# EsauPR/3d-pose-baseline

Measured on NVIDIA B200. Metric: poses/sec (fused MLP inference, bf16), higher is better.
Workload: dtype bf16

## Files before the change

3d-pose-baseline_b200/csrc/mlp_tc.cu:

```cuda
#include <cstdlib>

#include "common.cuh"
#include "ptx.cuh"

namespace p3d {

static std::atomic<unsigned long long> g_l2_set_aside[64];
int l2persist_acquire(int dev, size_t bytes) {
  if (dev < 0 || dev >= 64) return P3D_OK;
  if (g_l2_set_aside[dev].load(std::memory_order_acquire) >= bytes) return P3D_OK;
  P3D_CUDA(cudaDeviceSetLimit(cudaLimitPersistingL2CacheSize, bytes));
  g_l2_set_aside[dev].store(bytes, std::memory_order_release);
  return P3D_OK;
}
int l2persist_release(int dev) {
  if (dev < 0 || dev >= 64 || g_l2_set_aside[dev].load(std::memory_order_acquire) == 0) return P3D_OK;
  cudaCtxResetPersistingL2Cache();
  P3D_CUDA(cudaDeviceSetLimit(cudaLimitPersistingL2CacheSize, 0));
  g_l2_set_aside[dev].store(0, std::memory_order_release);
  return P3D_OK;
}

namespace tc {

using namespace ptx;

constexpr int BM = 128;
constexpr int BN = 256;
constexpr int BK = 64;
constexpr int A_BYTES = BM * BK * 2;
constexpr int OUT_BYTES = BM * 64 * 2;
constexpr int NTHREADS = 256;
constexpr int TMEM_COLS = 512;
constexpr int MAX_SLABS = 64;

template <int CG> struct Tile {
  static constexpr int STAGES = CG == 1 ? 4 : 6;
  static constexpr int BAR_BYTES = 1024;
  static constexpr int B_ROWS = BN / CG;
  static constexpr int B_BYTES = B_ROWS * BK * 2;
  static constexpr int SMEM_BYTES = 1024  + STAGES * (A_BYTES + B_BYTES) + OUT_BYTES + 2 * BN * 4 + BAR_BYTES;
  static_assert(SMEM_BYTES <= 232448, "exceeds the 227 KB of shared memory per CTA");
};

struct Params {
  int L;
  int nlayers;
  int out_n;
  int out_valid;
  int residual;
  int ntiles;
  long long B;
  long long act_half_rows;
  const float* bias;
  float* y;
};

__device__ __forceinline__ uint32_t pack_bf16x2(float a, float b) {
  __nv_bfloat162 v = __floats2bfloat162_rn(a, b);
  return *reinterpret_cast<uint32_t*>(&v);
}

__device__ __forceinline__ uint64_t desc_at(uint32_t smem_addr) {
  constexpr uint32_t hi = (1024u >> 4) | (1u << 14) | (2u << 29);
  const uint32_t lo = ((smem_addr >> 4) & 0x3FFFu) | (1u << 16);
  return (static_cast<uint64_t>(hi) << 32) | lo;
}

template <int CG>
__global__ void __launch_bounds__(NTHREADS, 1)
mlp_forward_tc_kernel(const __grid_constant__ CUtensorMap tm_x, const __grid_constant__ CUtensorMap tm_act,
                      const __grid_constant__ CUtensorMap tm_w, const __grid_constant__ CUtensorMap tm_wout,
                      const Params p) {
  using T = Tile<CG>;
  constexpr int STAGES = T::STAGES;
  constexpr int B_BYTES = T::B_BYTES;
  extern __shared__ uint8_t smem_raw[];
  uint8_t* smem = reinterpret_cast<uint8_t*>((reinterpret_cast<uintptr_t>(smem_raw) + 1023) & ~uintptr_t(1023));
  uint8_t* sA = smem;
  uint8_t* sB = smem + STAGES * A_BYTES;
  uint8_t* sOut = sB + STAGES * B_BYTES;
  float* sBiasAll = reinterpret_cast<float*>(sOut + OUT_BYTES);
  uint64_t* bars = reinterpret_cast<uint64_t*>(sBiasAll + 2 * BN);
  uint64_t* full = bars;
  uint64_t* empty = bars + STAGES;
  uint64_t* tfull = bars + 2 * STAGES;
  uint64_t* tempty = tfull + 2;
  uint64_t* stg_full = tempty + 2;
  uint64_t* stg_free = stg_full + 1;
  uint64_t* slab_done = stg_free + 1;
  uint32_t* tmem_slot = reinterpret_cast<uint32_t*>(slab_done + MAX_SLABS);

  const int warp = threadIdx.x >> 5;
  const int lane = threadIdx.x & 31;
  const uint32_t rank = (CG == 2) ? cluster_ctarank() : 0u;
  const bool leader = (rank == 0);
  const int group_id = blockIdx.x / CG, ngroups = gridDim.x / CG;
  const int ngtiles = (p.ntiles + CG - 1) / CG;

  if (threadIdx.x == 0) {
    tma_prefetch_desc(&tm_x); tma_prefetch_desc(&tm_act); tma_prefetch_desc(&tm_w); tma_prefetch_desc(&tm_wout);
    for (int s = 0; s < STAGES; ++s) { mbar_init(&full[s], 2); mbar_init(&empty[s], 1); }
    for (int a = 0; a < 2; ++a) { mbar_init(&tfull[a], 1); mbar_init(&tempty[a], 4 * CG); }
    mbar_init(stg_full, 4); mbar_init(stg_free, 1);
    for (int c = 0; c < MAX_SLABS; ++c) mbar_init(&slab_done[c], 1);
    fence_barrier_init();
  }
  if (warp == 2) {
    if (CG == 2) { tmem_alloc_2sm(tmem_slot, TMEM_COLS); tmem_relinquish_2sm(); }
    else { tmem_alloc(tmem_slot, TMEM_COLS); tmem_relinquish(); }
  }
  tc_fence_before();
  if (CG == 2) cluster_sync(); else __syncthreads();
  tc_fence_after();
  const uint32_t tmem_base = *tmem_slot;

  const int L = p.L;
  const int nlayers = p.nlayers;
  const int nk_hidden = L / BK;
  const int nchunks_hidden = L / BN;

  if (warp == 0 || warp == 2) {
    const bool prodA = (warp == 0);
    int stage = 0; uint32_t phase = 0; uint32_t dep_layers = 0;
    for (int gt = group_id; gt < ngtiles; gt += ngroups) {
      const int tile = gt * CG + static_cast<int>(rank);
      for (int l = 0; l < nlayers; ++l) {
        const bool first = (l == 0), last = (l == nlayers - 1);
        const int nk = first ? 1 : nk_hidden;
        const int nchunks = last ? 1 : nchunks_hidden;
        const CUtensorMap* tmA = first ? &tm_x : &tm_act;
        const int a_row = first ? tile * BM
                                : static_cast<int>(((l & 1) ? 0 : p.act_half_rows) + static_cast<long long>(blockIdx.x) * BM);
        const int b_rows = last ? p.out_n / CG : T::B_ROWS;
        const uint32_t bytes = prodA ? A_BYTES : b_rows * BK * 2;
        for (int c = 0; c < nchunks; ++c) {
          const int b_row = (last ? 0 : l * L + c * BN) + static_cast<int>(rank) * b_rows;
          for (int ks = 0; ks < nk; ++ks) {
            if (prodA && !first && c == 0) mbar_wait(&slab_done[ks], dep_layers & 1, 100 + l);
            mbar_wait(&empty[stage], phase ^ 1, 1);
            if (elect_one()) {
              if (CG == 1) {
                mbar_arrive_expect_tx(&full[stage], bytes);
                if (prodA) tma_load_2d_hint(sA + stage * A_BYTES, tmA, &full[stage], ks * BK, a_row, first ? kEvictFirst : kEvictLast);
                else       tma_load_2d_hint(sB + stage * B_BYTES, last ? &tm_wout : &tm_w, &full[stage], ks * BK, b_row, kEvictLast);
              } else {
                if (leader) mbar_arrive_expect_tx(&full[stage], 2 * bytes);
                if (prodA) tma_load_2d_2sm_hint(sA + stage * A_BYTES, tmA, &full[stage], ks * BK, a_row, first ? kEvictFirst : kEvictLast);
                else       tma_load_2d_2sm_hint(sB + stage * B_BYTES, last ? &tm_wout : &tm_w, &full[stage], ks * BK, b_row, kEvictLast);
              }
            }
            __syncwarp();
            if (++stage == STAGES) { stage = 0; phase ^= 1; }
          }
        }
        if (!first) ++dep_layers;
      }
    }
  } else if (warp == 1 && leader) {
    int stage = 0; uint32_t phase = 0; uint32_t q = 0;
    const uint32_t idesc_hidden = umma_idesc_bf16_f32(BM * CG, BN);
    const uint32_t idesc_out = umma_idesc_bf16_f32(BM * CG, p.out_n);
    const uint32_t a_base = smem_u32(sA), b_base = smem_u32(sB);
    for (int gt = group_id; gt < ngtiles; gt += ngroups) {
      for (int l = 0; l < nlayers; ++l) {
        const bool first = (l == 0), last = (l == nlayers - 1);
        const int nk = first ? 1 : nk_hidden;
        const int nchunks = last ? 1 : nchunks_hidden;
        const uint32_t idesc = last ? idesc_out : idesc_hidden;
        for (int c = 0; c < nchunks; ++c, ++q) {
          const uint32_t acc = q & 1, aphase = (q >> 1) & 1;
          mbar_wait(&tempty[acc], aphase ^ 1, 2);
          tc_fence_after();
          const uint32_t d_tmem = tmem_base + acc * BN;
          for (int ks = 0; ks < nk; ++ks) {
            mbar_wait(&full[stage], phase, 3);
            tc_fence_after();
            if (elect_one()) {
              const uint64_t ad = desc_at(a_base + stage * A_BYTES);
              const uint64_t bd = desc_at(b_base + stage * B_BYTES);
#pragma unroll
              for (int k = 0; k < BK / 16; ++k) {
                if (CG == 1) umma_bf16_ss(d_tmem, ad + 2 * k, bd + 2 * k, idesc, (ks | k) != 0 ? 1u : 0u);
                else         umma_bf16_ss_2sm(d_tmem, ad + 2 * k, bd + 2 * k, idesc, (ks | k) != 0 ? 1u : 0u);
              }
              if (CG == 1) {
                umma_commit(&empty[stage]);
                if (ks == nk - 1) umma_commit(&tfull[acc]);
              } else {
                umma_commit_2sm(&empty[stage], 0x3);
                if (ks == nk - 1) umma_commit_2sm(&tfull[acc], 0x3);
              }
            }
            __syncwarp();
            if (++stage == STAGES) { stage = 0; phase ^= 1; }
          }
        }
      }
    }
  } else if (warp == 3) {
    if (lane == 0) {
      uint32_t n = 0;
      for (int gt = group_id; gt < ngtiles; gt += ngroups) {
        for (int l = 0; l < nlayers - 1; ++l) {
          const bool to_p = (l == 0) || ((l & 1) == 0);
          const bool add_res = p.residual && l >= 2 && ((l & 1) == 0);
          const int drow = static_cast<int>((to_p ? 0 : p.act_half_rows) + static_cast<long long>(blockIdx.x) * BM);
          const int nsl = L / 64;
          for (int sl = 0; sl < nsl; ++sl, ++n) {
            mbar_wait(stg_full, n & 1, 6);
            if (add_res) tma_reduce_add_2d_hint(&tm_act, sOut, sl * 64, drow, kEvictLast);
            else         tma_store_2d_hint(&tm_act, sOut, sl * 64, drow, kEvictLast);
            tma_store_commit();
            tma_store_wait_read<0>();
            mbar_arrive(stg_free);
            if (sl > 0) { tma_store_wait<1>(); mbar_arrive(&slab_done[sl - 1]); }
          }
          tma_store_wait<0>();
          mbar_arrive(&slab_done[nsl - 1]);
        }
      }
    }
  } else if (warp >= 4) {
    const int ew = warp - 4;
    const int row = ew * 32 + lane;
    uint8_t* my_out = sOut + row * 128;
    uint32_t q = 0, nslab = 0;
    for (int gt = group_id; gt < ngtiles; gt += ngroups) {
      const int tile = gt * CG + static_cast<int>(rank);
      for (int l = 0; l < nlayers; ++l) {
        const bool last = (l == nlayers - 1);
        const int nchunks = last ? 1 : nchunks_hidden;
        for (int c = 0; c < nchunks; ++c, ++q) {
          const uint32_t acc = q & 1, aphase = (q >> 1) & 1;
          const int wrow0 = last ? (nlayers - 1) * L : l * L + c * BN;
          float* sBias = sBiasAll + (q & 1) * BN;
          sBias[row] = __ldg(p.bias + wrow0 + row);
          if (!last) sBias[row + 128] = __ldg(p.bias + wrow0 + row + 128);
          named_bar_sync(1, 128);
          mbar_wait(&tfull[acc], aphase, 4);
          tc_fence_after();
          const uint32_t taddr = tmem_base + (static_cast<uint32_t>(ew * 32) << 16) + acc * BN;
          if (!last) {
#pragma unroll 1
            for (int s = 0; s < BN / 64; ++s) {
              uint32_t v0[32], v1[32];
              tmem_ld_32x32b_x32(taddr + s * 64, v0);
              tmem_ld_32x32b_x32(taddr + s * 64 + 32, v1);
              tmem_ld_wait();
              if (s == BN / 64 - 1) {
                tc_fence_before();
                __syncwarp();
                if (lane == 0) { if (CG == 1) mbar_arrive(&tempty[acc]); else mbar_arrive_cluster(&tempty[acc], 0); }
              }
              uint32_t o[32];
              const float* bs = sBias + s * 64;
#pragma unroll
              for (int j = 0; j < 16; ++j) {
                o[j] = pack_bf16x2(fmaxf(__uint_as_float(v0[2 * j]) + bs[2 * j], 0.f),
                                   fmaxf(__uint_as_float(v0[2 * j + 1]) + bs[2 * j + 1], 0.f));
                o[16 + j] = pack_bf16x2(fmaxf(__uint_as_float(v1[2 * j]) + bs[32 + 2 * j], 0.f),
                                        fmaxf(__uint_as_float(v1[2 * j + 1]) + bs[32 + 2 * j + 1], 0.f));
              }
              mbar_wait(stg_free, (nslab & 1) ^ 1, 5);
#pragma unroll
              for (int j = 0; j < 8; ++j)
                *reinterpret_cast<uint4*>(my_out + ((j ^ (row & 7)) << 4)) = make_uint4(o[4 * j], o[4 * j + 1], o[4 * j + 2], o[4 * j + 3]);
              fence_proxy_async_smem();
              __syncwarp();
              if (lane == 0) mbar_arrive(stg_full);
              ++nslab;
            }
          } else {
            const long long grow = static_cast<long long>(tile) * BM + row;
            for (int g = 0; g < p.out_n / 16; ++g) {
              uint32_t v[16];
              tmem_ld_32x32b_x16(taddr + g * 16, v);
              tmem_ld_wait();
              if (grow < p.B) {
                float* yp = p.y + grow * p.out_valid + g * 16;
#pragma unroll
                for (int j = 0; j < 16; j += 2) {
                  const int col = g * 16 + j;
                  if (col + 1 < p.out_valid) {
                    float2 o2 = make_float2(__uint_as_float(v[j]) + sBias[col], __uint_as_float(v[j + 1]) + sBias[col + 1]);
                    __stcs(reinterpret_cast<float2*>(yp + j), o2);
                  } else if (col < p.out_valid) {
                    __stcs(yp + j, __uint_as_float(v[j]) + sBias[col]);
                  }
                }
              }
            }
            tc_fence_before();
            __syncwarp();
            if (lane == 0) { if (CG == 1) mbar_arrive(&tempty[acc]); else mbar_arrive_cluster(&tempty[acc], 0); }
          }
        }
      }
    }
  }

  tc_fence_before();
  if (CG == 2) cluster_sync(); else __syncthreads();
  if (warp == 2) {
    tc_fence_after();
    if (CG == 2) tmem_dealloc_2sm(tmem_base, TMEM_COLS); else tmem_dealloc(tmem_base, TMEM_COLS);
  }
}

constexpr int B_BYTES = BN * BK * 2;
__global__ void __launch_bounds__(128, 1)
umma_gemm_debug_kernel(const __grid_constant__ CUtensorMap tm_a, const __grid_constant__ CUtensorMap tm_w,
                       float* C, int N, int K) {
  extern __shared__ uint8_t smem_raw[];
  uint8_t* smem = reinterpret_cast<uint8_t*>((reinterpret_cast<uintptr_t>(smem_raw) + 1023) & ~uintptr_t(1023));
  uint8_t* sA = smem;
  uint8_t* sB = smem + A_BYTES;
  uint64_t* bar_full = reinterpret_cast<uint64_t*>(sB + B_BYTES);
  uint64_t* bar_mma = bar_full + 1;
  uint32_t* tmem_slot = reinterpret_cast<uint32_t*>(bar_mma + 1);
  const int warp = threadIdx.x >> 5, lane = threadIdx.x & 31;
  if (threadIdx.x == 0) { mbar_init(bar_full, 1); mbar_init(bar_mma, 1); fence_barrier_init(); }
  if (warp == 0) { tmem_alloc(tmem_slot, 256); tmem_relinquish(); }
  tc_fence_before(); __syncthreads(); tc_fence_after();
  const uint32_t tmem_base = *tmem_slot;
  if (threadIdx.x == 0) {
    const uint32_t idesc = umma_idesc_bf16_f32(128, N);
    for (int ks = 0; ks < K / BK; ++ks) {
      mbar_arrive_expect_tx(bar_full, A_BYTES + N * BK * 2);
      tma_load_2d(sA, &tm_a, bar_full, ks * BK, 0);
      tma_load_2d(sB, &tm_w, bar_full, ks * BK, 0);
      mbar_wait(bar_full, ks & 1, 10);
      tc_fence_after();
      for (int k = 0; k < BK / 16; ++k)
        umma_bf16_ss(tmem_base, umma_desc_k_sw128(smem_u32(sA) + k * 32), umma_desc_k_sw128(smem_u32(sB) + k * 32),
                     idesc, (ks | k) != 0 ? 1u : 0u);
      umma_commit(bar_mma);
      mbar_wait(bar_mma, ks & 1, 11);
    }
  }
  tc_fence_before(); __syncthreads(); tc_fence_after();
  const int row = warp * 32 + lane;
  for (int g = 0; g < N / 16; ++g) {
    uint32_t v[16];
    tmem_ld_32x32b_x16(tmem_base + (static_cast<uint32_t>(warp * 32) << 16) + g * 16, v);
    tmem_ld_wait();
    for (int j = 0; j < 16; ++j) C[row * N + g * 16 + j] = __uint_as_float(v[j]);
  }
  tc_fence_before(); __syncthreads();
  if (warp == 0) { tc_fence_after(); tmem_dealloc(tmem_base, 256); }
}

typedef CUresult (*EncodeTiledFn)(CUtensorMap*, CUtensorMapDataType, cuuint32_t, void*, const cuuint64_t*,
                                  const cuuint64_t*, const cuuint32_t*, const cuuint32_t*, CUtensorMapInterleave,
                                  CUtensorMapSwizzle, CUtensorMapL2promotion, CUtensorMapFloatOOBfill);

static EncodeTiledFn get_encode_fn() {
  static EncodeTiledFn fn = nullptr;
  if (!fn) {
    void* ptr = nullptr;
    cudaDriverEntryPointQueryResult qres;
    if (cudaGetDriverEntryPoint("cuTensorMapEncodeTiled", &ptr, cudaEnableDefault, &qres) != cudaSuccess ||
        qres != cudaDriverEntryPointSuccess)
      return nullptr;
    fn = reinterpret_cast<EncodeTiledFn>(ptr);
  }
  return fn;
}

static int make_tmap(CUtensorMap* out, const void* base, uint64_t rows, uint64_t cols, uint64_t pitch_elems,
                     uint32_t box_rows) {
  EncodeTiledFn fn = get_encode_fn();
  if (!fn) { set_error("cuTensorMapEncodeTiled entry point not available"); return P3D_ERR_CUDA; }
  cuuint64_t gdim[2] = {cols, rows};
  cuuint64_t gstride[1] = {pitch_elems * 2};
  cuuint32_t box[2] = {static_cast<cuuint32_t>(BK), box_rows};
  cuuint32_t estr[2] = {1, 1};
  CUresult r = fn(out, CU_TENSOR_MAP_DATA_TYPE_BFLOAT16, 2, const_cast<void*>(base), gdim, gstride, box, estr,
                  CU_TENSOR_MAP_INTERLEAVE_NONE, CU_TENSOR_MAP_SWIZZLE_128B, CU_TENSOR_MAP_L2_PROMOTION_L2_256B,
                  CU_TENSOR_MAP_FLOAT_OOB_FILL_NONE);
  if (r != CUDA_SUCCESS) { set_error("cuTensorMapEncodeTiled failed with CUresult %d", (int)r); return P3D_ERR_CUDA; }
  return P3D_OK;
}

template <int CG>
static int launch_forward(p3d_model* m, const __nv_bfloat16* xb, float* y, int64_t B, cudaStream_t st) {
  using T = Tile<CG>;
  const int L = m->L;
  const int ntiles = static_cast<int>((B + BM - 1) / BM);
  const int ngtiles = (ntiles + CG - 1) / CG;
  const int max_groups = m->num_sms / CG;
  const int grid = CG * (ngtiles < max_groups ? ngtiles : max_groups);
  const int nlayers = static_cast<int>(m->layers.size());
  const int out_n = (m->out_size + 15) / 16 * 16;
  CUtensorMap tm_x, tm_act, tm_w, tm_wout;
  P3D_TRY(make_tmap(&tm_x, xb, static_cast<uint64_t>(B), 64, 64, BM));
  P3D_TRY(make_tmap(&tm_act, m->act_scratch, 2ull * grid * BM, L, L, BM));
  P3D_TRY(make_tmap(&tm_w, m->wt_bf16, static_cast<uint64_t>(nlayers - 1) * L, m->kpad, m->kpad, T::B_ROWS));
  P3D_TRY(make_tmap(&tm_wout, m->wt_bf16 + static_cast<size_t>(nlayers - 1) * L * m->kpad, out_n, m->kpad, m->kpad, out_n / CG));
  Params p;
  p.L = L; p.nlayers = nlayers; p.out_n = out_n; p.out_valid = m->out_size; p.residual = m->cfg.residual;
  p.ntiles = ntiles; p.B = B; p.act_half_rows = static_cast<long long>(grid) * BM;
  p.bias = m->bias_fold; p.y = y;
  static PerDeviceOnce attr_set;
  if (attr_set.needed()) {
    P3D_CUDA(cudaFuncSetAttribute(mlp_forward_tc_kernel<CG>, cudaFuncAttributeMaxDynamicSharedMemorySize, T::SMEM_BYTES));
    attr_set.mark();
  }
  cudaLaunchConfig_t cfg{};
  cfg.gridDim = dim3(grid); cfg.blockDim = dim3(NTHREADS); cfg.dynamicSmemBytes = T::SMEM_BYTES; cfg.stream = st;
  cudaLaunchAttribute attr[2];
  attr[0].id = cudaLaunchAttributeClusterDimension;
  attr[0].val.clusterDim.x = CG; attr[0].val.clusterDim.y = 1; attr[0].val.clusterDim.z = 1;
  cfg.attrs = attr; cfg.numAttrs = 1;
  static const bool l2_persist = [] { const char* e = getenv("P3D_L2_PERSIST"); return !(e && e[0] == '0'); }();
  if (l2_persist) {
    int dev = 0, max_persist = 0, max_window = 0;
    P3D_CUDA(cudaGetDevice(&dev));
    P3D_CUDA(cudaDeviceGetAttribute(&max_persist, cudaDevAttrMaxPersistingL2CacheSize, dev));
    P3D_CUDA(cudaDeviceGetAttribute(&max_window, cudaDevAttrMaxAccessPolicyWindowSize, dev));
    const size_t scratch = sizeof(__nv_bfloat16) * 2ull * grid * BM * L;
    if (scratch <= static_cast<size_t>(max_persist) && scratch <= static_cast<size_t>(max_window)) {
      P3D_TRY(l2persist_acquire(dev, scratch));
      attr[1].id = cudaLaunchAttributeAccessPolicyWindow;
      attr[1].val.accessPolicyWindow.base_ptr = m->act_scratch;
      attr[1].val.accessPolicyWindow.num_bytes = scratch;
      attr[1].val.accessPolicyWindow.hitRatio = 1.0f;
      attr[1].val.accessPolicyWindow.hitProp = cudaAccessPropertyPersisting;
      attr[1].val.accessPolicyWindow.missProp = cudaAccessPropertyNormal;
      cfg.numAttrs = 2;
    }
  }
  cudaEvent_t e0 = nullptr, e1 = nullptr;
  if (prof::enabled()) prof::begin(st, &e0, &e1);
  P3D_CUDA(cudaLaunchKernelEx(&cfg, mlp_forward_tc_kernel<CG>, tm_x, tm_act, tm_w, tm_wout, p));
  P3D_LAUNCH_CHECK();
  if (e0) prof::end(st, e0, e1);
  return P3D_OK;
}

int forward_bf16(p3d_model* m, const __nv_bfloat16* xb, float* y, int64_t B, cudaStream_t st) {
  const int L = m->L;
  P3D_REQUIRE(L % BN == 0 && L / 64 <= MAX_SLABS, "bf16 tensor-core path needs linear_size %% 256 == 0 and <= 4096 (got %d)", L);
  if (m->act_grid < m->num_sms) {
    if (m->act_scratch) cudaFree(m->act_scratch);
    P3D_CUDA(cudaMalloc(&m->act_scratch, sizeof(__nv_bfloat16) * 2ull * m->num_sms * BM * L));
    m->act_grid = m->num_sms;
  }
  static int cg = -1;
  if (cg < 0) {
    const char* e = getenv("P3D_TC_CG");
    cg = (e && e[0] == '1') ? 1 : 2;
  }
  return cg == 1 ? launch_forward<1>(m, xb, y, B, st) : launch_forward<2>(m, xb, y, B, st);
}

int debug_umma_gemm(const void* A, const void* W, float* C, int N, int K, cudaStream_t st) {
  P3D_REQUIRE(N % 16 == 0 && N >= 16 && N <= 256 && K % 64 == 0 && K >= 64, "debug gemm: bad N=%d K=%d", N, K);
  CUtensorMap tm_a, tm_w;
  P3D_TRY(make_tmap(&tm_a, A, 128, K, K, 128));
  P3D_TRY(make_tmap(&tm_w, W, N, K, K, N));
  const int smem = 1024 + A_BYTES + B_BYTES + 64;
  P3D_CUDA(cudaFuncSetAttribute(umma_gemm_debug_kernel, cudaFuncAttributeMaxDynamicSharedMemorySize, smem));
  umma_gemm_debug_kernel<<<1, 128, smem, st>>>(tm_a, tm_w, C, N, K);
  P3D_LAUNCH_CHECK();
  return P3D_OK;
}

}
}
```

Before: 153.3 million.

## Widen epilogue to eight warps issuing their own TMA stores, drop store warp

Removes the dedicated TMA-store warp and the single shared output staging buffer. Eight epilogue warps now each own a small staging buffer and issue their own stores or reduce-adds per 32-row quarter, using a new 32-row tensor map. Each pair of warps splits the TMEM column slabs and software-pipelines the TMEM loads against the bias/ReLU/pack work. The goal is to take the store serialization and the stg_full/stg_free handshake off the critical path between layers. In exchange, pipeline stages drop by one to free shared memory, the thread count grows to 384, and optional clock64 stamp instrumentation is added behind an environment variable.

```diff
diff --git a/3d-pose-baseline_b200/csrc/mlp_tc.cu b/3d-pose-baseline_b200/csrc/mlp_tc.cu
--- a/3d-pose-baseline_b200/csrc/mlp_tc.cu
+++ b/3d-pose-baseline_b200/csrc/mlp_tc.cu
@@ -29,17 +29,20 @@
 constexpr int BN = 256;
 constexpr int BK = 64;
 constexpr int A_BYTES = BM * BK * 2;
-constexpr int OUT_BYTES = BM * 64 * 2;
-constexpr int NTHREADS = 256;
+constexpr int EPI_ROWS = 32;
+constexpr int STG_BYTES = EPI_ROWS * 64 * 2;
+constexpr int EPI_WARPS = 8;
+constexpr int NTHREADS = (4 + EPI_WARPS) * 32;
 constexpr int TMEM_COLS = 512;
 constexpr int MAX_SLABS = 64;
 
 template <int CG> struct Tile {
-  static constexpr int STAGES = CG == 1 ? 4 : 6;
+  static constexpr int STAGES = CG == 1 ? 3 : 5;
   static constexpr int BAR_BYTES = 1024;
   static constexpr int B_ROWS = BN / CG;
   static constexpr int B_BYTES = B_ROWS * BK * 2;
-  static constexpr int SMEM_BYTES = 1024  + STAGES * (A_BYTES + B_BYTES) + OUT_BYTES + 2 * BN * 4 + BAR_BYTES;
+  static constexpr int SMEM_BYTES = 1024  + STAGES * (A_BYTES + B_BYTES) + EPI_WARPS * STG_BYTES +
+                                    2 * BN * 4 + BAR_BYTES;
   static_assert(SMEM_BYTES <= 232448, "exceeds the 227 KB of shared memory per CTA");
 };
 
@@ -54,7 +57,19 @@
   long long act_half_rows;
   const float* bias;
   float* y;
+  unsigned long long* stamps;
 };
+
+constexpr int STAMP_SLOTS = 64;
+constexpr int STAMP_SPAN = 0;
+constexpr int STAMP_TILES = 1;
+constexpr int STAMP_EPI_STG = 2;
+constexpr int STAMP_EPI_TFULL = 3;
+constexpr int STAMP_MAX_LAYERS = 16;
+constexpr int STAMP_TEMPTY = 16;
+constexpr int STAMP_FULL = 32;
+constexpr int STAMP_SLAB = 48;
+__device__ __forceinline__ int stamp_layer(int l) { return l < STAMP_MAX_LAYERS ? l : STAMP_MAX_LAYERS - 1; }
 
 __device__ __forceinline__ uint32_t pack_bf16x2(float a, float b) {
   __nv_bfloat162 v = __floats2bfloat162_rn(a, b);
@@ -67,11 +82,11 @@
   return (static_cast<uint64_t>(hi) << 32) | lo;
 }
 
-template <int CG>
+template <int CG, bool STAMPS>
 __global__ void __launch_bounds__(NTHREADS, 1)
 mlp_forward_tc_kernel(const __grid_constant__ CUtensorMap tm_x, const __grid_constant__ CUtensorMap tm_act,
-                      const __grid_constant__ CUtensorMap tm_w, const __grid_constant__ CUtensorMap tm_wout,
-                      const Params p) {
+                      const __grid_constant__ CUtensorMap tm_act_st, const __grid_constant__ CUtensorMap tm_w,
+                      const __grid_constant__ CUtensorMap tm_wout, const Params p) {
   using T = Tile<CG>;
   constexpr int STAGES = T::STAGES;
   constexpr int B_BYTES = T::B_BYTES;
@@ -79,16 +94,14 @@
   uint8_t* smem = reinterpret_cast<uint8_t*>((reinterpret_cast<uintptr_t>(smem_raw) + 1023) & ~uintptr_t(1023));
   uint8_t* sA = smem;
   uint8_t* sB = smem + STAGES * A_BYTES;
-  uint8_t* sOut = sB + STAGES * B_BYTES;
-  float* sBiasAll = reinterpret_cast<float*>(sOut + OUT_BYTES);
+  uint8_t* sStg = sB + STAGES * B_BYTES;
+  float* sBiasAll = reinterpret_cast<float*>(sStg + EPI_WARPS * STG_BYTES);
   uint64_t* bars = reinterpret_cast<uint64_t*>(sBiasAll + 2 * BN);
   uint64_t* full = bars;
   uint64_t* empty = bars + STAGES;
   uint64_t* tfull = bars + 2 * STAGES;
   uint64_t* tempty = tfull + 2;
-  uint64_t* stg_full = tempty + 2;
-  uint64_t* stg_free = stg_full + 1;
-  uint64_t* slab_done = stg_free + 1;
+  uint64_t* slab_done = tempty + 2;
   uint32_t* tmem_slot = reinterpret_cast<uint32_t*>(slab_done + MAX_SLABS);
 
   const int warp = threadIdx.x >> 5;
@@ -97,13 +110,16 @@
   const bool leader = (rank == 0);
   const int group_id = blockIdx.x / CG, ngroups = gridDim.x / CG;
   const int ngtiles = (p.ntiles + CG - 1) / CG;
+  unsigned long long* stamps = STAMPS ? p.stamps + static_cast<size_t>(blockIdx.x) * STAMP_SLOTS : nullptr;
+  long long t_entry = 0;
+  if constexpr (STAMPS) t_entry = clock64();
 
   if (threadIdx.x == 0) {
-    tma_prefetch_desc(&tm_x); tma_prefetch_desc(&tm_act); tma_prefetch_desc(&tm_w); tma_prefetch_desc(&tm_wout);
+    tma_prefetch_desc(&tm_x); tma_prefetch_desc(&tm_act); tma_prefetch_desc(&tm_act_st);
+    tma_prefetch_desc(&tm_w); tma_prefetch_desc(&tm_wout);
     for (int s = 0; s < STAGES; ++s) { mbar_init(&full[s], 2); mbar_init(&empty[s], 1); }
-    for (int a = 0; a < 2; ++a) { mbar_init(&tfull[a], 1); mbar_init(&tempty[a], 4 * CG); }
-    mbar_init(stg_full, 4); mbar_init(stg_free, 1);
-    for (int c = 0; c < MAX_SLABS; ++c) mbar_init(&slab_done[c], 1);
+    for (int a = 0; a < 2; ++a) { mbar_init(&tfull[a], 1); mbar_init(&tempty[a], EPI_WARPS * CG); }
+    for (int c = 0; c < MAX_SLABS; ++c) mbar_init(&slab_done[c], 4);
     fence_barrier_init();
   }
   if (warp == 2) {
@@ -129,6 +145,7 @@
         const bool first = (l == 0), last = (l == nlayers - 1);
         const int nk = first ? 1 : nk_hidden;
         const int nchunks = last ? 1 : nchunks_hidden;
+        long long w_slab = 0;
         const CUtensorMap* tmA = first ? &tm_x : &tm_act;
         const int a_row = first ? tile * BM
                                 : static_cast<int>(((l & 1) ? 0 : p.act_half_rows) + static_cast<long long>(blockIdx.x) * BM);
@@ -137,7 +154,12 @@
         for (int c = 0; c < nchunks; ++c) {
           const int b_row = (last ? 0 : l * L + c * BN) + static_cast<int>(rank) * b_rows;
           for (int ks = 0; ks < nk; ++ks) {
-            if (prodA && !first && c == 0) mbar_wait(&slab_done[ks], dep_layers & 1, 100 + l);
+            if (prodA && !first && c == 0) {
+              long long t0 = 0;
+              if constexpr (STAMPS) t0 = clock64();
+              mbar_wait(&slab_done[ks], dep_layers & 1, 100 + l);
+              if constexpr (STAMPS) w_slab += clock64() - t0;
+            }
             mbar_wait(&empty[stage], phase ^ 1, 1);
             if (elect_one()) {
               if (CG == 1) {
@@ -155,6 +177,7 @@
           }
         }
         if (!first) ++dep_layers;
+        if constexpr (STAMPS) if (prodA && lane == 0 && w_slab) atomicAdd(stamps + STAMP_SLAB + stamp_layer(l), static_cast<unsigned long long>(w_slab));
       }
     }
   } else if (warp == 1 && leader) {
@@ -168,13 +191,18 @@
         const int nk = first ? 1 : nk_hidden;
         const int nchunks = last ? 1 : nchunks_hidden;
         const uint32_t idesc = last ? idesc_out : idesc_hidden;
+        long long w_te = 0, w_full = 0, t0 = 0;
         for (int c = 0; c < nchunks; ++c, ++q) {
           const uint32_t acc = q & 1, aphase = (q >> 1) & 1;
+          if constexpr (STAMPS) t0 = clock64();
           mbar_wait(&tempty[acc], aphase ^ 1, 2);
+          if constexpr (STAMPS) w_te += clock64() - t0;
           tc_fence_after();
           const uint32_t d_tmem = tmem_base + acc * BN;
           for (int ks = 0; ks < nk; ++ks) {
+            if constexpr (STAMPS) t0 = clock64();
             mbar_wait(&full[stage], phase, 3);
+            if constexpr (STAMPS) w_full += clock64() - t0;
             tc_fence_after();
             if (elect_one()) {
               const uint64_t ad = desc_at(a_base + stage * A_BYTES);
@@ -196,84 +224,99 @@
             if (++stage == STAGES) { stage = 0; phase ^= 1; }
           }
         }
-      }
-    }
-  } else if (warp == 3) {
-    if (lane == 0) {
-      uint32_t n = 0;
-      for (int gt = group_id; gt < ngtiles; gt += ngroups) {
-        for (int l = 0; l < nlayers - 1; ++l) {
-          const bool to_p = (l == 0) || ((l & 1) == 0);
-          const bool add_res = p.residual && l >= 2 && ((l & 1) == 0);
-          const int drow = static_cast<int>((to_p ? 0 : p.act_half_rows) + static_cast<long long>(blockIdx.x) * BM);
-          const int nsl = L / 64;
-          for (int sl = 0; sl < nsl; ++sl, ++n) {
-            mbar_wait(stg_full, n & 1, 6);
-            if (add_res) tma_reduce_add_2d_hint(&tm_act, sOut, sl * 64, drow, kEvictLast);
-            else         tma_store_2d_hint(&tm_act, sOut, sl * 64, drow, kEvictLast);
-            tma_store_commit();
-            tma_store_wait_read<0>();
-            mbar_arrive(stg_free);
-            if (sl > 0) { tma_store_wait<1>(); mbar_arrive(&slab_done[sl - 1]); }
-          }
-          tma_store_wait<0>();
-          mbar_arrive(&slab_done[nsl - 1]);
+        if constexpr (STAMPS) if (lane == 0) {
+          atomicAdd(stamps + STAMP_TEMPTY + stamp_layer(l), static_cast<unsigned long long>(w_te));
+          atomicAdd(stamps + STAMP_FULL + stamp_layer(l), static_cast<unsigned long long>(w_full));
         }
       }
     }
   } else if (warp >= 4) {
     const int ew = warp - 4;
-    const int row = ew * 32 + lane;
-    uint8_t* my_out = sOut + row * 128;
-    uint32_t q = 0, nslab = 0;
+    const int qd = warp & 3;
+    const int half = ew >> 2;
+    const int row = qd * 32 + lane;
+    uint8_t* buf = sStg + ew * STG_BYTES;
+    uint32_t q = 0;
+    long long w_stg = 0, w_tfull = 0, t0 = 0;
     for (int gt = group_id; gt < ngtiles; gt += ngroups) {
       const int tile = gt * CG + static_cast<int>(rank);
+      if constexpr (STAMPS) if (threadIdx.x == 128) atomicAdd(stamps + STAMP_TILES, 1ull);
       for (int l = 0; l < nlayers; ++l) {
         const bool last = (l == nlayers - 1);
         const int nchunks = last ? 1 : nchunks_hidden;
+        const bool to_p = (l == 0) || ((l & 1) == 0);
+        const bool add_res = p.residual && l >= 2 && ((l & 1) == 0);
+        const int drow = static_cast<int>((to_p ? 0 : p.act_half_rows) + static_cast<long long>(blockIdx.x) * BM) + qd * EPI_ROWS;
         for (int c = 0; c < nchunks; ++c, ++q) {
           const uint32_t acc = q & 1, aphase = (q >> 1) & 1;
           const int wrow0 = last ? (nlayers - 1) * L : l * L + c * BN;
           float* sBias = sBiasAll + (q & 1) * BN;
-          sBias[row] = __ldg(p.bias + wrow0 + row);
-          if (!last) sBias[row + 128] = __ldg(p.bias + wrow0 + row + 128);
-          named_bar_sync(1, 128);
+          const int bi = ew * 32 + lane;
+          if (!last || bi < BM) sBias[bi] = __ldg(p.bias + wrow0 + bi);
+          named_bar_sync(1, EPI_WARPS * 32);
+          if constexpr (STAMPS) t0 = clock64();
           mbar_wait(&tfull[acc], aphase, 4);
+          if constexpr (STAMPS) w_tfull += clock64() - t0;
           tc_fence_after();
-          const uint32_t taddr = tmem_base + (static_cast<uint32_t>(ew * 32) << 16) + acc * BN;
+          const uint32_t taddr = tmem_base + (static_cast<uint32_t>(qd * 32) << 16) + acc * BN;
           if (!last) {
+            uint32_t v0[32], v1[32];
+            tmem_ld_32x32b_x32(taddr + half * 64, v0);
 #pragma unroll 1
-            for (int s = 0; s < BN / 64; ++s) {
-              uint32_t v0[32], v1[32];
-              tmem_ld_32x32b_x32(taddr + s * 64, v0);
+            for (int s = half; s < BN / 64; s += 2) {
+              tmem_ld_wait();
               tmem_ld_32x32b_x32(taddr + s * 64 + 32, v1);
+              uint32_t o[32];
+              const float* bs = sBias + s * 64;
+#pragma unroll
+              for (int j = 0; j < 16; ++j)
+                o[j] = pack_bf16x2(fmaxf(__uint_as_float(v0[2 * j]) + bs[2 * j], 0.f),
+                                   fmaxf(__uint_as_float(v0[2 * j + 1]) + bs[2 * j + 1], 0.f));
               tmem_ld_wait();
-              if (s == BN / 64 - 1) {
+              if (s + 2 < BN / 64) {
+                tmem_ld_32x32b_x32(taddr + (s + 2) * 64, v0);
+              } else {
                 tc_fence_before();
                 __syncwarp();
                 if (lane == 0) { if (CG == 1) mbar_arrive(&tempty[acc]); else mbar_arrive_cluster(&tempty[acc], 0); }
               }
-              uint32_t o[32];
-              const float* bs = sBias + s * 64;
 #pragma unroll
-              for (int j = 0; j < 16; ++j) {
-                o[j] = pack_bf16x2(fmaxf(__uint_as_float(v0[2 * j]) + bs[2 * j], 0.f),
-                                   fmaxf(__uint_as_float(v0[2 * j + 1]) + bs[2 * j + 1], 0.f));
+              for (int j = 0; j < 16; ++j)
                 o[16 + j] = pack_bf16x2(fmaxf(__uint_as_float(v1[2 * j]) + bs[32 + 2 * j], 0.f),
                                         fmaxf(__uint_as_float(v1[2 * j + 1]) + bs[32 + 2 * j + 1], 0.f));
-              }
-              mbar_wait(stg_free, (nslab & 1) ^ 1, 5);
+              if (lane == 0) {
+                if constexpr (STAMPS) t0 = clock64();
+                tma_store_wait_read<0>();
+                if constexpr (STAMPS) w_stg += clock64() - t0;
+              }
+              __syncwarp();
 #pragma unroll
               for (int j = 0; j < 8; ++j)
-                *reinterpret_cast<uint4*>(my_out + ((j ^ (row & 7)) << 4)) = make_uint4(o[4 * j], o[4 * j + 1], o[4 * j + 2], o[4 * j + 3]);
+                *reinterpret_cast<uint4*>(buf + lane * 128 + ((j ^ (lane & 7)) << 4)) = make_uint4(o[4 * j], o[4 * j + 1], o[4 * j + 2], o[4 * j + 3]);
               fence_proxy_async_smem();
               __syncwarp();
-              if (lane == 0) mbar_arrive(stg_full);
-              ++nslab;
+              if (lane == 0) {
+                const int sl = c * (BN / 64) + s;
+                if (add_res) tma_reduce_add_2d_hint(&tm_act_st, buf, sl * 64, drow, kEvictLast);
+                else         tma_store_2d_hint(&tm_act_st, buf, sl * 64, drow, kEvictLast);
+                tma_store_commit();
+                if (sl >= 2) {
+                  if constexpr (STAMPS) t0 = clock64();
+                  tma_store_wait<1>();
+                  if constexpr (STAMPS) w_stg += clock64() - t0;
+                  mbar_arrive(&slab_done[sl - 2]);
+                }
+              }
+            }
+            if (c == nchunks - 1 && lane == 0) {
+              if constexpr (STAMPS) t0 = clock64();
+              tma_store_wait<0>();
+              if constexpr (STAMPS) w_stg += clock64() - t0;
+              mbar_arrive(&slab_done[L / 64 - 2 + half]);
             }
           } else {
             const long long grow = static_cast<long long>(tile) * BM + row;
-            for (int g = 0; g < p.out_n / 16; ++g) {
+            for (int g = half; g < p.out_n / 16; g += 2) {
               uint32_t v[16];
               tmem_ld_32x32b_x16(taddr + g * 16, v);
               tmem_ld_wait();
@@ -298,10 +341,15 @@
         }
       }
     }
+    if constexpr (STAMPS) if (lane == 0) {
+      atomicAdd(stamps + STAMP_EPI_STG, static_cast<unsigned long long>(w_stg));
+      atomicAdd(stamps + STAMP_EPI_TFULL, static_cast<unsigned long long>(w_tfull));
+    }
   }
 
   tc_fence_before();
   if (CG == 2) cluster_sync(); else __syncthreads();
+  if constexpr (STAMPS) if (threadIdx.x == 0) stamps[STAMP_SPAN] = static_cast<unsigned long long>(clock64() - t_entry);
   if (warp == 2) {
     tc_fence_after();
     if (CG == 2) tmem_dealloc_2sm(tmem_base, TMEM_COLS); else tmem_dealloc(tmem_base, TMEM_COLS);
@@ -383,8 +431,9 @@
   return P3D_OK;
 }
 
-template <int CG>
-static int launch_forward(p3d_model* m, const __nv_bfloat16* xb, float* y, int64_t B, cudaStream_t st) {
+template <int CG, bool STAMPS>
+static int launch_forward(p3d_model* m, const __nv_bfloat16* xb, float* y, int64_t B, cudaStream_t st,
+                          unsigned long long* stamps) {
   using T = Tile<CG>;
   const int L = m->L;
   const int ntiles = static_cast<int>((B + BM - 1) / BM);
@@ -393,18 +442,19 @@
   const int grid = CG * (ngtiles < max_groups ? ngtiles : max_groups);
   const int nlayers = static_cast<int>(m->layers.size());
   const int out_n = (m->out_size + 15) / 16 * 16;
-  CUtensorMap tm_x, tm_act, tm_w, tm_wout;
+  CUtensorMap tm_x, tm_act, tm_act_st, tm_w, tm_wout;
   P3D_TRY(make_tmap(&tm_x, xb, static_cast<uint64_t>(B), 64, 64, BM));
   P3D_TRY(make_tmap(&tm_act, m->act_scratch, 2ull * grid * BM, L, L, BM));
+  P3D_TRY(make_tmap(&tm_act_st, m->act_scratch, 2ull * grid * BM, L, L, EPI_ROWS));
   P3D_TRY(make_tmap(&tm_w, m->wt_bf16, static_cast<uint64_t>(nlayers - 1) * L, m->kpad, m->kpad, T::B_ROWS));
   P3D_TRY(make_tmap(&tm_wout, m->wt_bf16 + static_cast<size_t>(nlayers - 1) * L * m->kpad, out_n, m->kpad, m->kpad, out_n / CG));
   Params p;
   p.L = L; p.nlayers = nlayers; p.out_n = out_n; p.out_valid = m->out_size; p.residual = m->cfg.residual;
   p.ntiles = ntiles; p.B = B; p.act_half_rows = static_cast<long long>(grid) * BM;
-  p.bias = m->bias_fold; p.y = y;
+  p.bias = m->bias_fold; p.y = y; p.stamps = stamps;
   static PerDeviceOnce attr_set;
   if (attr_set.needed()) {
-    P3D_CUDA(cudaFuncSetAttribute(mlp_forward_tc_kernel<CG>, cudaFuncAttributeMaxDynamicSharedMemorySize, T::SMEM_BYTES));
+    P3D_CUDA(cudaFuncSetAttribute(mlp_forward_tc_kernel<CG, STAMPS>, cudaFuncAttributeMaxDynamicSharedMemorySize, T::SMEM_BYTES));
     attr_set.mark();
   }
   cudaLaunchConfig_t cfg{};
@@ -433,7 +483,7 @@
   }
   cudaEvent_t e0 = nullptr, e1 = nullptr;
   if (prof::enabled()) prof::begin(st, &e0, &e1);
-  P3D_CUDA(cudaLaunchKernelEx(&cfg, mlp_forward_tc_kernel<CG>, tm_x, tm_act, tm_w, tm_wout, p));
+  P3D_CUDA(cudaLaunchKernelEx(&cfg, mlp_forward_tc_kernel<CG, STAMPS>, tm_x, tm_act, tm_act_st, tm_w, tm_wout, p));
   P3D_LAUNCH_CHECK();
   if (e0) prof::end(st, e0, e1);
   return P3D_OK;
@@ -452,7 +502,11 @@
     const char* e = getenv("P3D_TC_CG");
     cg = (e && e[0] == '1') ? 1 : 2;
   }
-  return cg == 1 ? launch_forward<1>(m, xb, y, B, st) : launch_forward<2>(m, xb, y, B, st);
+  if (const char* e = getenv("P3D_TC_STAMPS")) {
+    auto* s = reinterpret_cast<unsigned long long*>(strtoull(e, nullptr, 0));
+    if (s) return cg == 1 ? launch_forward<1, true>(m, xb, y, B, st, s) : launch_forward<2, true>(m, xb, y, B, st, s);
+  }
+  return cg == 1 ? launch_forward<1, false>(m, xb, y, B, st, nullptr) : launch_forward<2, false>(m, xb, y, B, st, nullptr);
 }
 
 int debug_umma_gemm(const void* A, const void* W, float* C, int N, int K, cudaStream_t st) {
```

Result: no change. 154.0 million (median of 6 runs) (+0.4%).
